# pjmikkol/bwtc

Measured on AMD Instinct MI355X. Metric: MB/s compressed (BWT+encode) on 256 MiB block, higher is better.
Workload: dtype u8/u32/u64 integer

## Files before the change

bwtc_amd/csrc/wavelet_encoder.hip:

```cpp
#include "bwt_engine.hpp"
#include "entropy_host.hpp"
#include "wavelet_host.hpp"
#include "wavelet_pipeline.hpp"
#include <algorithm>
#include <chrono>
#include <future>
#include <cstdio>
#include <cstdlib>
#include <cstring>
#include <map>
#include <memory>
#include <utility>
#include <vector>

namespace bwtc_hip {

static u32 device_model_rejects(const u32* h_tail, u32 n_coded, bool state_ok) {
  u32 r = 0;
  if (h_tail[1]) r |= BWTC_HIP_REJECT_FLAGS;
  if (h_tail[2] != n_coded) r |= BWTC_HIP_REJECT_COUNT;
  if (h_tail[3]) r |= BWTC_HIP_REJECT_SCAN;
  if (!state_ok) r |= BWTC_HIP_REJECT_STATE;
  if (std::getenv("BWTC_HIP_TEST_MODELS_FALLBACK")) r |= BWTC_HIP_REJECT_TEST;
  return r;
// ... 375 lines not shown
    e.prob_free.back()->swap(job.prob);
  }
  *out_bytes = job.record.size();
  const int rc = job.failed ? -2 : job.record.size() <= job.user_cap ? 0 : -1;
  if (e.pipeline) {
    std::shared_ptr<WaveletJob> last(std::move(jobp));
    e.pipeline->dispose(std::move(last));
  }
  return rc;
}

int wavelet_join_begun(BwtEngine& e) {
  if (!e.deferred_queue) return 0;
  for (std::map<u64, std::shared_ptr<DeviceWaveletJob> >::iterator it = e.jobs.begin(); it != e.jobs.end(); ++it) {
    if (it->second->queued) continue;
    const int rc = wavelet_encode_queue(e, it->first, e.wavelet_state, &e.wavelet_state);
    if (rc) return rc;
  }
  return 0;
}

void wavelet_pipeline_release(BwtEngine& e) {
  (void)wavelet_join_begun(e);
  e.half_job.reset();
  e.copy_job.reset();
  for (std::map<u64, std::shared_ptr<DeviceWaveletJob> >::iterator it = e.jobs.begin(); it != e.jobs.end(); ++it)
    if (it->second->queued) HostPipeline::wait(*it->second);
  e.jobs.clear();
  if (e.pipeline && std::getenv("BWTC_HIP_DEBUG") && e.pipeline->clock.blocks)
    std::fprintf(stderr, "wavelet pipeline: %llu blocks; host time in models %.3f s, in range coders %.3f s (summed over threads)\n",
                 (unsigned long long)e.pipeline->clock.blocks.load(), e.pipeline->clock.model_ns.load() * 1e-9,
                 e.pipeline->clock.coder_ns.load() * 1e-9);
  if (e.pipeline && std::getenv("BWTC_HIP_DEBUG") && e.pipeline->clock.scalar_ns.load())
    std::fprintf(stderr, "wavelet pipeline: %.3f s of the range coders' time in the scalar tasks of the longest sections, the rest in the lane engines\n",
                 e.pipeline->clock.scalar_ns.load() * 1e-9);
  delete e.pipeline;
  e.pipeline = nullptr;
  e.codes_pool.clear();
  e.w_pool.clear();
  e.prob_free.clear();
}

}
```

bwtc_amd/csrc/wavelet_pipeline.cpp:

```cpp
#include "wavelet_pipeline.hpp"

#include <algorithm>
#include <cstdio>
#include <cstdlib>
#include <cstring>

namespace bwtc_hip {

namespace {
unsigned envNumber(const char* name, unsigned fallback) {
  const char* v = std::getenv(name);
  return v && std::atoi(v) > 0 ? static_cast<unsigned>(std::atoi(v)) : fallback;
}
uint64_t since(const std::chrono::steady_clock::time_point& t0) {
  return static_cast<uint64_t>(std::chrono::duration_cast<std::chrono::nanoseconds>(std::chrono::steady_clock::now() - t0).count());
}
}

HostPipeline::HostPipeline(unsigned threads, uint64_t huge_group_elements, unsigned depth)
    : groups_(), pool_(threads), huge_(huge_group_elements) {
  const unsigned P = pool_.size();
  const char* force = std::getenv("BWTC_HIP_CODER_LANES");
  const bool lanes = bwtc::wavelet::simdCoderAvailable() && (force ? force[0] == '1' : depth >= kLaneDepth);
  coder_tasks_ = envNumber("BWTC_HIP_CODER_TASKS", 2);
  max_engines_ = std::max(1u, envNumber("BWTC_HIP_MODEL_ENGINES", lanes ? (P * 7 + 15) / 16 : (P + 3) / 4));
  max_coder_engines_ = lanes ? envNumber("BWTC_HIP_CODER_ENGINES", std::max(1u, (P * 6 + 15) / 16)) : 0u;
  long_chain_ = static_cast<uint64_t>(std::getenv("BWTC_HIP_LONG_CHAIN_MI") ? std::atoi(std::getenv("BWTC_HIP_LONG_CHAIN_MI")) : 0) << 20;
  if (std::getenv("BWTC_HIP_LONG_CHAIN_ELEMENTS")) long_chain_ = std::strtoull(std::getenv("BWTC_HIP_LONG_CHAIN_ELEMENTS"), nullptr, 10);
  if (long_chain_ == 0) long_chain_ = ~static_cast<uint64_t>(0);
  max_pair_engines_ = lanes && long_chain_ != ~static_cast<uint64_t>(0) ? envNumber("BWTC_HIP_PAIR_ENGINES", std::max(1u, (P * 3 + 7) / 8)) : 0u;
  const char* fforce = std::getenv("BWTC_HIP_FUSED");
  const bool fused = bwtc::wavelet::simdCoderAvailable() && bwtc::wavelet::simdModelsAvailable() &&
                     (fforce ? fforce[0] == '1' : depth >= kFusedDepth);
  max_fused_engines_ = fused ? envNumber("BWTC_HIP_FUSED_ENGINES", P) : 0u;
  groups_.on_block_modelled = [this](const std::shared_ptr<WaveletJob>& j) { submitSections(j); };
  chains_.on_block_coded = [this](WaveletJob& j) { finish(j); };
  fused_sections_.on_block_coded = [this](WaveletJob& j) { finish(j); };
  long_chains_.on_block_coded = [this](WaveletJob& j) { finish(j); };
  w_chains_.on_block_coded = [this](WaveletJob& j) { finish(j); };
  w_long_chains_.on_block_coded = [this](WaveletJob& j) { finish(j); };
  max_w_engines_ = bwtc::wavelet::simdCoderAvailable() ? envNumber("BWTC_HIP_W_ENGINES", std::max(1u, P / 4)) : 0u;
  if (std::getenv("BWTC_HIP_W_ENGINES") && std::atoi(std::getenv("BWTC_HIP_W_ENGINES")) == 0) max_w_engines_ = 0;
  max_w_pair_engines_ = envNumber("BWTC_HIP_W_PAIR_ENGINES", 0);
  w_lanes_ = envNumber("BWTC_HIP_W_LANES", 16);
  w_long_chain_ = static_cast<uint64_t>(envNumber("BWTC_HIP_W_LONG_MI", 8)) << 20;
  if (std::getenv("BWTC_HIP_LONG_CHAIN_ELEMENTS")) w_long_chain_ = std::strtoull(std::getenv("BWTC_HIP_LONG_CHAIN_ELEMENTS"), nullptr, 10);
}

HostPipeline::~HostPipeline() {}

void HostPipeline::wait(WaveletJob& job) {
  std::unique_lock<std::mutex> g(job.mu);
  job.cv.wait(g, [&] { return job.done; });
}

bool HostPipeline::waitFor(WaveletJob& job, unsigned milliseconds) {
  std::unique_lock<std::mutex> g(job.mu);
  return job.cv.wait_for(g, std::chrono::milliseconds(milliseconds), [&] { return job.done; });
}

void HostPipeline::finishNow(WaveletJob& job) {
  std::vector<uint8_t>& rec = job.record;
  size_t total = rec.size();
  for (size_t s = 0; s < job.outs.size(); ++s) total += job.outs[s].bytes.size();
  rec.reserve(total);
  for (size_t s = 0; s < job.outs.size(); ++s) rec.insert(rec.end(), job.outs[s].bytes.begin(), job.outs[s].bytes.end());
  const uint64_t len = rec.size() - 6;
  for (int i = 0; i < 6; ++i) rec[i] = static_cast<uint8_t>(len >> (8 * (5 - i)));
  if (job.user_out && rec.size() <= job.user_cap) std::memcpy(job.user_out, rec.data(), rec.size());
  job.t_finished = std::chrono::steady_clock::now();
  { std::lock_guard<std::mutex> g(job.mu); job.done = true; job.cv.notify_all(); }
}

void HostPipeline::finish(WaveletJob& job) {
  --clock.unfinished;
  finishNow(job);
  if (job.t_begun.time_since_epoch().count())
    clock.latency_ns += static_cast<uint64_t>(std::chrono::duration_cast<std::chrono::nanoseconds>(job.t_finished - job.t_begun).count());
  ++clock.finished;
// ... 15 lines not shown
  std::vector<std::function<void()> > next;
  const uint64_t longest = std::max<uint64_t>(1, jobp->coder->largestSectionElements());
  const size_t balanced = static_cast<size_t>(std::min<uint64_t>(pool_.size(), jobp->coder->elements() / longest));
  const size_t engines = std::max<size_t>(1, std::min<size_t>(std::max(coder_tasks_, balanced), (jobp->coder->sectionTasks() + 1) / 2));
  for (size_t q = 0; q < engines; ++q) {
    next.push_back([this, jobp] {
      WaveletJob& j = *jobp;
      const auto t0 = std::chrono::steady_clock::now();
      const size_t did = j.coder->codeSectionsPaired(&j.section_cursor, j.prob.data(), &j.outs);
      clock.coder_ns += since(t0);
      bool fin;
      { std::lock_guard<std::mutex> g(j.mu); j.sections_left -= did; fin = did > 0 && j.sections_left == 0; }
      if (fin) finish(j);
    });
  }
  pool_.submit(jobp->rank, next);
}

uint32_t HostPipeline::queue(const std::shared_ptr<WaveletJob>& jobp, uint32_t fsm8_state, char model, const uint32_t* expect_end) {
  WaveletJob& job = *jobp;
  noteBegin();
  if (job.w) {
    job.coder.reset(new bwtc::wavelet::StreamCoder(job.plan, job.coded_pos.data(), job.w_end_state, bwtc::wavelet::StreamCoder::Modelled()));
    freshOutputs(job, job.plan.sections.size());
    job.t_queued = job.t_modelled = std::chrono::steady_clock::now();
    job.models_left = 0;
    job.sections_left = job.coder->sectionTasks();
    ++clock.blocks;
    if (job.sections_left == 0) { finishNow(job); ++clock.finished; return job.w_end_state; }
    ++clock.unfinished;
    if (std::getenv("BWTC_HIP_DEBUG")) {
      std::fprintf(stderr, "w-route: %zu sections, elements (Mi):", job.coder->sectionTasks());
      for (size_t k = 0; k < job.coder->sectionTasks() && k < 12; ++k) std::fprintf(stderr, " %.1f", job.coder->sectionElements(k) / 1048576.0);
      std::fprintf(stderr, " ...; %u lane engines at most, scalar from %.0f Mi\n", max_w_engines_, w_long_chain_ / 1048576.0);
    }
    if (max_w_engines_) {
      const uint64_t cut = std::max<uint64_t>(w_long_chain_, job.coder->largestSectionElements() / 5);
      size_t n_long = 0;
      while (n_long < job.coder->sectionTasks() && job.coder->sectionElements(n_long) >= cut) ++n_long;
      std::vector<std::function<void()> > own;
      if (max_w_pair_engines_ && n_long) {
        if (w_long_chains_.add(jobp, 0, n_long, max_w_pair_engines_))
          pool_.submit(0, [this] { bwtc::wavelet::runCoderLanes(w_long_chains_, 2, &clock.coder_ns); });
      } else
      for (size_t k = 0; k < n_long; ++k) {
        own.push_back([this, jobp, k] {
          WaveletJob& j = *jobp;
          const auto t0 = std::chrono::steady_clock::now();
          j.coder->codeSectionW(k, j.w, &j.outs);
          const uint64_t dt = since(t0);
          clock.coder_ns += dt;
          clock.scalar_ns += dt;
          bool fin;
          { std::lock_guard<std::mutex> g(j.mu); fin = --j.sections_left == 0; }
          if (fin) finish(j);
        });
      }
      if (!own.empty()) pool_.submit(job.rank, own);
      if (w_chains_.add(jobp, n_long, job.coder->sectionTasks(), max_w_engines_))
        pool_.submit(0, [this] { bwtc::wavelet::runCoderLanes(w_chains_, static_cast<int>(w_lanes_), &clock.coder_ns); });
      return job.w_end_state;
    }
    const uint64_t longest = std::max<uint64_t>(1, job.coder->largestSectionElements());
    const size_t balanced = static_cast<size_t>(std::min<uint64_t>(pool_.size(), (job.coder->elements() + longest - 1) / longest));
    const size_t engines = std::max<size_t>(1, std::min<size_t>(std::max<size_t>(2, balanced), job.coder->sectionTasks()));
    std::vector<std::function<void()> > next;
    for (size_t q = 0; q < engines; ++q) {
      next.push_back([this, jobp] {
        WaveletJob& j = *jobp;
        const auto t0 = std::chrono::steady_clock::now();
        const size_t did = j.coder->codeSectionsW(&j.section_cursor, j.w, &j.outs);
        clock.coder_ns += since(t0);
// ... 71 lines not shown
```

bwtc_amd/csrc/wavelet_pipeline.hpp:

```cpp
#pragma once
#include <malloc.h>
#include <atomic>
#include <chrono>
#include <condition_variable>
#include <cstdint>
#include <cstdlib>
#include <deque>
#include <functional>
#include <map>
#include <memory>
#include <mutex>
#include <thread>
#include <vector>

#include <pthread.h>
#include <sched.h>
#include <sys/resource.h>
#include <sys/syscall.h>
#include <unistd.h>

#include "wavelet_host.hpp"

namespace bwtc_hip {

struct StageClock {
  std::atomic<uint64_t> model_ns{0}, coder_ns{0}, blocks{0}, finished{0};
  std::atomic<uint64_t> scalar_ns{0};
  std::atomic<uint64_t> latency_ns{0};
  std::atomic<int> unfinished{0};
};

struct WaveletRoutes {
  std::atomic<uint64_t> trees_device{0}, trees_host{0};
  std::atomic<uint64_t> models_device{0}, models_rejected{0}, lost_turn{0};
// ... 85 lines not shown
  bool next(bwtc::wavelet::ModelGroupDesc* d, int prefer);
  void done(void* cookie);
  bool retire(int prefer) {
    std::lock_guard<std::mutex> g(mu_);
    if (!queue_.empty()) return false;
    --engines_[prefer];
    return true;
  }
  std::function<void(const std::shared_ptr<WaveletJob>&)> on_block_modelled;
 private:
  struct Entry { std::shared_ptr<WaveletJob> job; std::vector<uint32_t> list[2]; size_t at[2]; };
  std::mutex mu_;
  std::deque<Entry> queue_;
  unsigned engines_[3];
};

class BlockChainSource : public bwtc::wavelet::ChainSource {
 public:
  BlockChainSource() : engines_(0) {}
  bool add(const std::shared_ptr<WaveletJob>& job, size_t first, size_t last, unsigned max_engines);
  bool next(bwtc::wavelet::ChainDesc* d);
  void done(void* cookie);
  bool retire() {
    std::lock_guard<std::mutex> g(mu_);
    if (!queue_.empty()) return false;
    --engines_;
    return true;
  }
  std::function<void(WaveletJob&)> on_block_coded;
 private:
  struct Entry { std::shared_ptr<WaveletJob> job; size_t at, end; };
  std::mutex mu_;
  std::deque<Entry> queue_;
  unsigned engines_;
};

class BlockSectionSource : public bwtc::wavelet::SectionSource {
 public:
  BlockSectionSource() : engines_(0) {}
  bool add(const std::shared_ptr<WaveletJob>& job, unsigned max_engines);
  bool next(bwtc::wavelet::FusedSectionDesc* d);
  void done(void* cookie);
  bool retire() {
    std::lock_guard<std::mutex> g(mu_);
    if (!queue_.empty()) return false;
    --engines_;
    return true;
  }
  std::function<void(WaveletJob&)> on_block_coded;
 private:
  struct Entry { std::shared_ptr<WaveletJob> job; size_t at; };
  std::mutex mu_;
  std::deque<Entry> queue_;
  unsigned engines_;
};

struct WaveletJob : std::enable_shared_from_this<WaveletJob> {
  virtual ~WaveletJob() {}
  std::vector<uint8_t> record;
  bwtc::wavelet::StreamPlan plan;
  std::vector<uint32_t> coded_pos;
  const uint8_t* codes = nullptr;
  RawBuffer<uint16_t> prob;
  std::unique_ptr<bwtc::wavelet::StreamCoder> coder;
  std::vector<bwtc::wavelet::SectionOutput> outs;
  std::vector<std::vector<bwtc::wavelet::FusedGroup> > fused_groups;
// ... 68 lines not shown
    const uint64_t now = static_cast<uint64_t>(std::chrono::duration_cast<std::chrono::nanoseconds>(
        std::chrono::steady_clock::now().time_since_epoch()).count());
    const uint64_t last = last_begin_ns_.exchange(now);
    if (last && now > last) {
      const uint64_t d = now - last, old = begin_interval_ns_.load();
      begin_interval_ns_.store(old ? (old * 7 + d) / 8 : d);
    }
  }
  StageClock clock;
  WaveletRoutes* routes = nullptr;
 private:
  std::atomic<uint64_t> last_begin_ns_{0}, begin_interval_ns_{0};
  enum { kSpares = 40 };
  std::atomic<uint32_t> disposed_{0};
  std::mutex spare_mu_;
  std::vector<std::vector<bwtc::wavelet::SectionOutput> > spare_outs_;
  std::vector<std::vector<uint8_t> > spare_records_;
  void freshOutputs(WaveletJob& job, size_t n) {
    if (job.outs.empty()) takeSpareOutputs(&job.outs);
    job.outs.resize(n);
    for (size_t s = 0; s < n; ++s) job.outs[s].bytes.clear();
  }
  void submitSections(const std::shared_ptr<WaveletJob>& job);
  void finish(WaveletJob& job);
  BlockGroupSource groups_;
  BlockChainSource chains_;
  BlockChainSource long_chains_;
  BlockChainSource w_chains_;
  BlockChainSource w_long_chains_;
  unsigned max_w_pair_engines_;
  unsigned w_lanes_;
  unsigned max_w_engines_;
  uint64_t w_long_chain_;
  BlockSectionSource fused_sections_;
  WorkerPool pool_;
  uint64_t huge_;
  unsigned max_engines_;
  unsigned max_coder_engines_;
  unsigned max_pair_engines_;
  uint64_t long_chain_;
  unsigned max_fused_engines_;
  size_t coder_tasks_;
};

inline int BlockGroupSource::add(const std::shared_ptr<WaveletJob>& job, size_t first_group, unsigned max_engines) {
  Entry e;
  e.job = job;
  e.at[0] = e.at[1] = 0;
  for (size_t k = first_group; k < job->coder->modelTasks(); ++k)
    e.list[job->coder->taskIsInteger(k) ? 0 : 1].push_back(static_cast<uint32_t>(k));
  std::lock_guard<std::mutex> g(mu_);
  queue_.push_back(std::move(e));
  if (engines_[1] + engines_[2] >= max_engines) return 0;
  const int prefer = engines_[1] * 2 < engines_[2] || (engines_[2] > 0 && engines_[1] == 0 && max_engines > 1) ? 1 : 2;
  ++engines_[prefer];
  return prefer;
}

inline bool BlockGroupSource::next(bwtc::wavelet::ModelGroupDesc* d, int prefer) {
  std::shared_ptr<WaveletJob> job;
  size_t k = 0;
  {
    std::lock_guard<std::mutex> g(mu_);
    while (!queue_.empty() && queue_.front().at[0] >= queue_.front().list[0].size() &&
           queue_.front().at[1] >= queue_.front().list[1].size())
      queue_.pop_front();
// ... 23 lines not shown
  e.at = first;
  e.end = last;
  std::lock_guard<std::mutex> g(mu_);
  queue_.push_back(std::move(e));
  if (engines_ >= max_engines) return false;
  ++engines_;
  return true;
}

inline bool BlockChainSource::next(bwtc::wavelet::ChainDesc* d) {
  std::shared_ptr<WaveletJob> job;
  size_t k = 0;
  {
    std::lock_guard<std::mutex> g(mu_);
    while (!queue_.empty() && queue_.front().at >= queue_.front().end) queue_.pop_front();
    if (queue_.empty()) return false;
    job = queue_.front().job;
    k = queue_.front().at++;
  }
  if (job->w) job->coder->describeChainW(k, job->w, &job->outs, d);
  else job->coder->describeChain(k, job->prob.data(), &job->outs, d);
  d->cookie = job.get();
  return true;
}

inline void BlockChainSource::done(void* cookie) {
  WaveletJob* job = static_cast<WaveletJob*>(cookie);
  const std::shared_ptr<WaveletJob> keep = job->shared_from_this();
  bool last;
  { std::lock_guard<std::mutex> g(job->mu); last = --job->sections_left == 0; }
  if (last) on_block_coded(*job);
}

inline bool BlockSectionSource::add(const std::shared_ptr<WaveletJob>& job, unsigned max_engines) {
  Entry e;
  e.job = job;
  e.at = 0;
  std::lock_guard<std::mutex> g(mu_);
  queue_.push_back(std::move(e));
  if (engines_ >= max_engines) return false;
  ++engines_;
  return true;
}

inline bool BlockSectionSource::next(bwtc::wavelet::FusedSectionDesc* d) {
  std::shared_ptr<WaveletJob> job;
  size_t k = 0;
  {
    std::lock_guard<std::mutex> g(mu_);
    while (!queue_.empty() && queue_.front().at >= queue_.front().job->coder->sectionTasks()) queue_.pop_front();
    if (queue_.empty()) return false;
    job = queue_.front().job;
    k = queue_.front().at++;
  }
  job->coder->describeSectionFused(k, &job->outs, &job->fused_groups[k], d);
  d->cookie = job.get();
  return true;
}

inline void BlockSectionSource::done(void* cookie) {
  WaveletJob* job = static_cast<WaveletJob*>(cookie);
  const std::shared_ptr<WaveletJob> keep = job->shared_from_this();
  bool last;
  { std::lock_guard<std::mutex> g(job->mu); last = --job->sections_left == 0; }
  if (last) on_block_coded(*job);
}
// ... 10 lines not shown
```

bwtc_amd/csrc/wavelet_rc.cpp:

```cpp
#include "wavelet_rc.hpp"

#include <immintrin.h>

#include <algorithm>
#include <chrono>
#include <cstdlib>
#include <cstring>

namespace bwtc {
namespace wavelet {
namespace {

inline uint32_t codeAt(const uint8_t* codes, uint64_t i) { return (codes[i >> 2] >> ((i & 3) * 2)) & 3u; }

}

void runChain(CoderChain& c, const uint8_t* codes, const uint16_t* prob, uint64_t until) {
  const uint64_t kChunk = 16384;
  uint32_t lo = c.lo, size = c.size;
  uint64_t b = c.i;
  for (; b < until; b += kChunk) {
    const uint64_t ce = std::min(until, b + kChunk);
    uint8_t* o = c.room(kChunk);
#define BWTC_RC_STEP(bit_, p_)                                                                          \
    {                                                                                                    \
      const uint32_t bit = (bit_);                                                                       \
      const uint32_t t = static_cast<uint32_t>((static_cast<uint64_t>(size) * (p_) + 2048u) >> 12);      \
      lo = bit ? lo : lo + t + 1;                                                                        \
      size = bit ? t - 1 : size - t - 1;                                                                 \
      while (((lo ^ (lo + size + 1)) & 0xFF000000u) == 0) { *o++ = static_cast<uint8_t>(lo >> 24); lo <<= 8; size = (size << 8) + 510u; } \
    }
    uint64_t i = b;
    for (; i < ce && (i & 3); ++i) BWTC_RC_STEP(codeAt(codes, i) & 1u, prob[i]);
    for (; i + 4 <= ce; i += 4) {
      const uint32_t four = codes[i >> 2];
      BWTC_RC_STEP(four & 1u, prob[i]);
      BWTC_RC_STEP((four >> 2) & 1u, prob[i + 1]);
      BWTC_RC_STEP((four >> 4) & 1u, prob[i + 2]);
      BWTC_RC_STEP((four >> 6) & 1u, prob[i + 3]);
    }
    for (; i < ce; ++i) BWTC_RC_STEP(codeAt(codes, i) & 1u, prob[i]);
#undef BWTC_RC_STEP
    c.used = static_cast<size_t>(o - c.out->data());
  }
  c.lo = lo; c.size = size; c.i = std::max(c.i, until);
}

void runChainW(CoderChain& c, const uint16_t* w, uint64_t until) {
  const uint64_t kChunk = 16384;
  uint32_t lo = c.lo, size = c.size;
  uint64_t b = c.i;
  for (; b < until; b += kChunk) {
    const uint64_t ce = std::min(until, b + kChunk);
    uint8_t* o = c.room(kChunk);
    for (uint64_t i = b; i < ce; ++i) {
      const uint32_t x = w[i];
      const uint32_t bit = x >> 15, m = x & 0x7FFFu;
      const uint32_t ns = static_cast<uint32_t>((static_cast<int64_t>(static_cast<uint64_t>(size) * m) + (static_cast<int64_t>(bit) - 2049)) >> 12);
      lo += (bit - 1u) & (size - ns);
      size = ns;
      while (((lo ^ (lo + size + 1)) & 0xFF000000u) == 0) { *o++ = static_cast<uint8_t>(lo >> 24); lo <<= 8; size = (size << 8) + 510u; }
    }
    c.used = static_cast<size_t>(o - c.out->data());
  }
  c.lo = lo; c.size = size; c.i = std::max(c.i, until);
}

void runChainPair(CoderChain& a, const uint8_t* codes_a, const uint16_t* prob_a,
                  CoderChain& b, const uint8_t* codes_b, const uint16_t* prob_b, uint64_t limit) {
  const uint64_t kChunk = 8192;
  uint64_t left = std::min(limit, std::min(a.e - a.i, b.e - b.i));
  while (left > 0) {
    const uint64_t n = std::min(left, kChunk);
    uint8_t* oa = a.room(kChunk);
    uint8_t* ob = b.room(kChunk);
    uint32_t loa = a.lo, sa = a.size, lob = b.lo, sb = b.size;
    uint64_t ia = a.i, ib = b.i;
#define BWTC_RC_FREE(lo, size, o, i, codes, prob)                                                         \
    {                                                                                                      \
      const uint32_t bit = codeAt(codes, i) & 1u;                                                          \
      const uint32_t t = static_cast<uint32_t>((static_cast<uint64_t>(size) * prob[i] + 2048u) >> 12);     \
      lo = bit ? lo : lo + t + 1;                                                                          \
      size = bit ? t - 1 : size - t - 1;                                                                   \
      const uint32_t same = ((lo ^ (lo + size + 1)) & 0xFF000000u) == 0;                                   \
      *o = static_cast<uint8_t>(lo >> 24);                                                                 \
      o += same;                                                                                           \
      lo = same ? lo << 8 : lo;                                                                            \
      size = same ? (size << 8) + 510u : size;                                                             \
      while (__builtin_expect(same && ((lo ^ (lo + size + 1)) & 0xFF000000u) == 0, 0)) { *o++ = static_cast<uint8_t>(lo >> 24); lo <<= 8; size = (size << 8) + 510u; } \
      ++i;                                                                                                 \
    }
    for (uint64_t k = 0; k < n; ++k) {
      BWTC_RC_FREE(loa, sa, oa, ia, codes_a, prob_a)
      BWTC_RC_FREE(lob, sb, ob, ib, codes_b, prob_b)
    }
#undef BWTC_RC_FREE
    a.lo = loa; a.size = sa; a.i = ia; a.used = static_cast<size_t>(oa - a.out->data());
    b.lo = lob; b.size = sb; b.i = ib; b.used = static_cast<size_t>(ob - b.out->data());
    left -= n;
  }
}

void runChainPairW(CoderChain& a, const uint16_t* wa, CoderChain& b, const uint16_t* wb, uint64_t limit) {
  const uint64_t kChunk = 8192;
  uint64_t left = std::min(limit, std::min(a.e - a.i, b.e - b.i));
  while (left > 0) {
    const uint64_t n = std::min(left, kChunk);
    uint8_t* oa = a.room(kChunk);
    uint8_t* ob = b.room(kChunk);
    uint32_t loa = a.lo, sa = a.size, lob = b.lo, sb = b.size;
    uint64_t ia = a.i, ib = b.i;
#define BWTC_RC_W(lo, size, o, i, w)                                                                      \
    {                                                                                                      \
      const uint32_t x = w[i];                                                                             \
      const uint32_t bit = x >> 15, m = x & 0x7FFFu;                                                       \
      const uint32_t ns = static_cast<uint32_t>((static_cast<int64_t>(static_cast<uint64_t>(size) * m) + (static_cast<int64_t>(bit) - 2049)) >> 12); \
      lo += (bit - 1u) & (size - ns);                                                                      \
      size = ns;                                                                                           \
      while (((lo ^ (lo + size + 1)) & 0xFF000000u) == 0) { *o++ = static_cast<uint8_t>(lo >> 24); lo <<= 8; size = (size << 8) + 510u; } \
      ++i;                                                                                                 \
    }
    for (uint64_t k = 0; k < n; ++k) {
      BWTC_RC_W(loa, sa, oa, ia, wa)
      BWTC_RC_W(lob, sb, ob, ib, wb)
    }
#undef BWTC_RC_W
    a.lo = loa; a.size = sa; a.i = ia; a.used = static_cast<size_t>(oa - a.out->data());
    b.lo = lob; b.size = sb; b.i = ib; b.used = static_cast<size_t>(ob - b.out->data());
    left -= n;
  }
}

void runChainPair(CoderChain& a, CoderChain& b, const uint8_t* codes, const uint16_t* prob) {
  runChainPair(a, codes, prob, b, codes, prob, ~static_cast<uint64_t>(0));
}

namespace {

const int kLanes = 16;
const uint64_t kScalarOnly = 512;
const int kMinLanes = 4;
const uint64_t kMaxWords = 512;

const int kGroups = 2;
const int kAll = kLanes * kGroups;

struct Lanes {
  alignas(64) uint32_t lo[kAll], size[kAll];
  const uint8_t* codes[kAll];
  const uint16_t* prob[kAll];
  uint64_t i[kAll];
  uint8_t* out[kAll];
  uint32_t advance[kAll];
};

alignas(64) const uint16_t kZeroProb[32] = {0};
alignas(64) const uint8_t kZeroCodes[8] = {0};

#define BWTC_AVX512 __attribute__((target("avx512f,avx512bw,avx512vl,avx512dq")))

BWTC_AVX512 inline void transpose16(__m512i r[16]) {
  __m512i t[16];
  for (int i = 0; i < 16; i += 2) { t[i] = _mm512_unpacklo_epi32(r[i], r[i + 1]); t[i + 1] = _mm512_unpackhi_epi32(r[i], r[i + 1]); }
  for (int i = 0; i < 16; i += 4) {
    r[i] = _mm512_unpacklo_epi64(t[i], t[i + 2]); r[i + 1] = _mm512_unpackhi_epi64(t[i], t[i + 2]);
    r[i + 2] = _mm512_unpacklo_epi64(t[i + 1], t[i + 3]); r[i + 3] = _mm512_unpackhi_epi64(t[i + 1], t[i + 3]);
  }
  for (int i = 0; i < 16; i += 8)
    for (int j = 0; j < 4; ++j) {
      t[i + j] = _mm512_shuffle_i32x4(r[i + j], r[i + j + 4], 0x88);
      t[i + j + 4] = _mm512_shuffle_i32x4(r[i + j], r[i + j + 4], 0xdd);
    }
  for (int j = 0; j < 8; ++j) {
    r[j] = _mm512_shuffle_i32x4(t[j], t[j + 8], 0x88);
    r[j + 8] = _mm512_shuffle_i32x4(t[j], t[j + 8], 0xdd);
  }
}

template <bool WMODE, int G>
BWTC_AVX512 void runWords(Lanes& L, uint64_t words, uint32_t busy_mask) {
  __m512i lo[G], size[G];
  __mmask16 kBusy[G];
  for (int g = 0; g < G; ++g) {
    lo[g] = _mm512_load_si512(L.lo + g * kLanes);
    size[g] = _mm512_load_si512(L.size + g * kLanes);
    kBusy[g] = static_cast<__mmask16>(busy_mask >> (g * kLanes));
  }
  const __m512i one = _mm512_set1_epi32(1), c4095 = _mm512_set1_epi32(4095), c2048 = _mm512_set1_epi32(2048);
  const __m512i top = _mm512_set1_epi32(static_cast<int>(0xFF000000u)), c510 = _mm512_set1_epi32(510);
  const __m512i lane0 = _mm512_slli_epi32(_mm512_setr_epi32(0, 1, 2, 3, 4, 5, 6, 7, 8, 9, 10, 11, 12, 13, 14, 15), 8);
  const __m512i c32768 = _mm512_set1_epi32(32768), c32767 = _mm512_set1_epi32(32767), cm2049 = _mm512_set1_epi32(-2049);
  alignas(64) uint32_t cw[kAll] = {0};
  alignas(64) uint32_t ev[G][16 * kLanes * 4 + 64];
  alignas(64) __m512i P[G][16];
  for (uint64_t w = 0; w < words; ++w) {
    for (int g = 0; g < G; ++g) {
      for (int l = 0; l < kLanes; ++l) {
        const int a = g * kLanes + l;
        P[g][l] = _mm512_cvtepu16_epi32(_mm256_loadu_si256(reinterpret_cast<const __m256i*>(L.prob[a] + L.i[a])));
        if (!WMODE) std::memcpy(&cw[a], L.codes[a] + (L.i[a] >> 2), 4);
        L.i[a] += L.advance[a];
      }
      transpose16(P[g]);
    }
    __m512i W[G];
    uint32_t n[G];
    for (int g = 0; g < G; ++g) { W[g] = _mm512_load_si512(cw + g * kLanes); n[g] = 0; }
    for (int t = 0; t < 16; ++t) {
#pragma GCC unroll 2
      for (int g = 0; g < G; ++g) {
        __m512i p = P[g][t];
        __mmask16 kBit;
        const __m512i hi = _mm512_srli_epi32(size[g], 12), lw = _mm512_and_si512(size[g], c4095);
        if (WMODE) {
          kBit = _mm512_test_epi32_mask(p, c32768);
          const __m512i m = _mm512_and_si512(p, c32767);
          __m512i c = _mm512_add_epi32(_mm512_mullo_epi32(lw, m), cm2049);
          c = _mm512_mask_add_epi32(c, kBit, c, one);
          const __m512i ns = _mm512_add_epi32(_mm512_mullo_epi32(hi, m), _mm512_srai_epi32(c, 12));
          lo[g] = _mm512_mask_add_epi32(lo[g], static_cast<__mmask16>(~kBit), lo[g], _mm512_sub_epi32(size[g], ns));
          size[g] = ns;
        } else {
          kBit = _mm512_test_epi32_mask(W[g], one);
          W[g] = _mm512_srli_epi32(W[g], 2);
          const __m512i tt = _mm512_add_epi32(_mm512_mullo_epi32(hi, p),
                                              _mm512_srli_epi32(_mm512_add_epi32(_mm512_mullo_epi32(lw, p), c2048), 12));
          const __m512i t1 = _mm512_add_epi32(tt, one);
          lo[g] = _mm512_mask_add_epi32(lo[g], static_cast<__mmask16>(~kBit), lo[g], t1);
          size[g] = _mm512_mask_blend_epi32(kBit, _mm512_sub_epi32(size[g], t1), _mm512_sub_epi32(tt, one));
        }
        __m512i hiend = _mm512_add_epi32(_mm512_add_epi32(lo[g], size[g]), one);
        __mmask16 m = _mm512_mask_testn_epi32_mask(kBusy[g], _mm512_xor_si512(lo[g], hiend), top);
        for (;;) {
          _mm512_storeu_si512(ev[g] + n[g], _mm512_maskz_compress_epi32(m, _mm512_or_si512(_mm512_srli_epi32(lo[g], 24), lane0)));
          n[g] += static_cast<uint32_t>(__builtin_popcount(m));
          lo[g] = _mm512_mask_slli_epi32(lo[g], m, lo[g], 8);
          size[g] = _mm512_mask_add_epi32(size[g], m, _mm512_slli_epi32(size[g], 8), c510);
          hiend = _mm512_add_epi32(_mm512_add_epi32(lo[g], size[g]), one);
          m = _mm512_mask_testn_epi32_mask(m, _mm512_xor_si512(lo[g], hiend), top);
          if (__builtin_expect(m == 0, 1)) break;
        }
      }
    }
    for (int g = 0; g < G; ++g)
      for (uint32_t k = 0; k < n[g]; ++k) { const uint32_t e = ev[g][k]; *L.out[g * kLanes + (e >> 8)]++ = static_cast<uint8_t>(e); }
  }
  for (int g = 0; g < G; ++g) {
    _mm512_store_si512(L.lo + g * kLanes, lo[g]);
    _mm512_store_si512(L.size + g * kLanes, size[g]);
  }
}

}

bool simdCoderAvailable() {
  static const bool ok = [] {
    const char* off = std::getenv("BWTC_HIP_SIMD");
    if (off && off[0] == '0') return false;
    off = std::getenv("BWTC_HIP_CODER_LANES");
    if (off && off[0] == '0') return false;
    return __builtin_cpu_supports("avx512f") && __builtin_cpu_supports("avx512bw") &&
           __builtin_cpu_supports("avx512vl") && __builtin_cpu_supports("avx512dq");
  }();
  return ok;
}

void runCoderLanes(ChainSource& src, int max_lanes, std::atomic<uint64_t>* busy_ns) {
  auto tick = std::chrono::steady_clock::now();
  auto account = [&] {
    if (!busy_ns) return;
    const auto now = std::chrono::steady_clock::now();
    *busy_ns += static_cast<uint64_t>(std::chrono::duration_cast<std::chrono::nanoseconds>(now - tick).count());
    tick = now;
  };
  const int lanes = std::max(1, std::min(max_lanes, kAll));
  const bool two = lanes > kLanes;
  Lanes L;
  CoderChain chain[kAll];
  ChainDesc desc[kAll];
  bool busy[kAll];
  for (int l = 0; l < kAll; ++l) busy[l] = false;
  bool sourceDry = false;
  bool wmode = false;
  auto scalar = [&](int l, uint64_t until) {
    if (desc[l].w) runChainW(chain[l], desc[l].w, until); else runChain(chain[l], desc[l].codes, desc[l].prob, until);
  };
  auto finishLane = [&](int l) {
    CoderChain& c = chain[l];
    scalar(l, c.e);
    c.finish();
    src.done(desc[l].cookie);
    busy[l] = false;
  };
  for (;;) {
    int nbusy = 0;
    for (int l = 0; l < lanes; ++l) {
      while (!busy[l] && !sourceDry) {
        if (!src.next(&desc[l])) { sourceDry = true; break; }
        CoderChain& c = chain[l];
        c.start(desc[l].begin, desc[l].end, desc[l].out);
        wmode = desc[l].w != nullptr;
        const uint64_t aligned = (c.i + 15) & ~static_cast<uint64_t>(15);
        busy[l] = true;
        if (c.e - c.i < kScalarOnly || aligned + 16 > c.e) { finishLane(l); continue; }
        scalar(l, aligned);
      }
      nbusy += busy[l];
    }
    account();
    if (nbusy == 0) {
      if (sourceDry && src.retire()) return;
      sourceDry = false;
      continue;
    }
    if (lanes < kMinLanes || (nbusy < kMinLanes && sourceDry)) {
      const uint64_t kSlice = static_cast<uint64_t>(1) << 22;
      int ids[kAll], n = 0;
      for (int l = 0; l < kAll; ++l) if (busy[l]) ids[n++] = l;
      if (n >= 2) {
        const int a = ids[0], b = ids[1];
        if (desc[a].w && desc[b].w) runChainPairW(chain[a], desc[a].w, chain[b], desc[b].w, kSlice);
        else if (desc[a].w || desc[b].w) { scalar(a, std::min(chain[a].e, chain[a].i + kSlice)); scalar(b, std::min(chain[b].e, chain[b].i + kSlice)); }
        else runChainPair(chain[a], desc[a].codes, desc[a].prob, chain[b], desc[b].codes, desc[b].prob, kSlice);
        if (chain[a].i >= chain[a].e) finishLane(a);
        if (chain[b].i >= chain[b].e) finishLane(b);
      } else {
        CoderChain& c = chain[ids[0]];
        scalar(ids[0], std::min(c.e, c.i + kSlice));
        if (c.i >= c.e) finishLane(ids[0]);
      }
      sourceDry = false;
      continue;
    }
    uint64_t words = kMaxWords;
    uint32_t mask = 0;
    for (int l = 0; l < kAll; ++l) if (busy[l]) { words = std::min(words, (chain[l].e - chain[l].i) >> 4); mask |= 1u << l; }
    if (words > 0) {
      for (int l = 0; l < kAll; ++l) {
        if (busy[l]) {
          CoderChain& c = chain[l];
          L.lo[l] = c.lo; L.size[l] = c.size; L.codes[l] = desc[l].codes; L.prob[l] = wmode ? desc[l].w : desc[l].prob; L.i[l] = c.i;
          L.out[l] = c.room(words * 16); L.advance[l] = 16;
        } else {
          L.lo[l] = 0; L.size[l] = 0xFFFFFFFEu; L.codes[l] = kZeroCodes; L.prob[l] = kZeroProb; L.i[l] = 0;
          L.out[l] = nullptr; L.advance[l] = 0;
        }
      }
      if (two && (mask >> kLanes)) { if (wmode) runWords<true, 2>(L, words, mask); else runWords<false, 2>(L, words, mask); }
      else { if (wmode) runWords<true, 1>(L, words, mask); else runWords<false, 1>(L, words, mask); }
      for (int l = 0; l < kAll; ++l) {
        if (!busy[l]) continue;
        CoderChain& c = chain[l];
        c.lo = L.lo[l]; c.size = L.size[l]; c.i = L.i[l];
        c.used = static_cast<size_t>(L.out[l] - c.out->data());
      }
    }
    for (int l = 0; l < kAll; ++l)
      if (busy[l] && chain[l].e - chain[l].i < 16) finishLane(l);
    sourceDry = false;
  }
}

}
}
```

bwtc_amd/csrc/wavelet_rc.hpp:

```cpp
#pragma once
#include <atomic>
#include <cstddef>
#include <cstdint>
#include <vector>

namespace bwtc {
namespace wavelet {

struct CoderChain {
  uint32_t lo, size;
  uint64_t i, e;
  std::vector<uint8_t>* out;
  size_t used;
  void start(uint64_t b, uint64_t end, std::vector<uint8_t>* o) {
    lo = 0; size = 0xFFFFFFFEu; i = b; e = end; out = o; used = o->size();
    if (end - b >= (1u << 16)) o->reserve(used + (end - b) / 7 + 4096);
  }
  uint8_t* room(uint64_t elements) {
    if (out->size() - used < 4 * elements + 8) out->resize(used + 4 * elements + 8 + out->size() / 2);
    return out->data() + used;
  }
  void finish() {
    out->resize(used + 4);
    uint8_t* o = out->data() + used;
    o[0] = static_cast<uint8_t>(lo >> 24); o[1] = 255; o[2] = 255; o[3] = 255;
  }
};

void runChain(CoderChain& c, const uint8_t* codes, const uint16_t* prob, uint64_t until);
void runChainW(CoderChain& c, const uint16_t* w, uint64_t until);
void runChainPairW(CoderChain& a, const uint16_t* wa, CoderChain& b, const uint16_t* wb, uint64_t limit);
void runChainPair(CoderChain& a, CoderChain& b, const uint8_t* codes, const uint16_t* prob);
void runChainPair(CoderChain& a, const uint8_t* codes_a, const uint16_t* prob_a,
                  CoderChain& b, const uint8_t* codes_b, const uint16_t* prob_b, uint64_t limit);

struct ChainDesc {
  const uint8_t* codes;
  const uint16_t* prob;
  uint64_t begin, end;
  std::vector<uint8_t>* out;
  void* cookie;
  const uint16_t* w = nullptr;
};

class ChainSource {
 public:
  virtual ~ChainSource() {}
  virtual bool next(ChainDesc* c) = 0;
  virtual void done(void* cookie) = 0;
  virtual bool retire() { return true; }
};

bool simdCoderAvailable();

void runCoderLanes(ChainSource& src, int max_lanes = 16, std::atomic<uint64_t>* busy_ns = nullptr);

}
}
```

Baseline: 5877.

## Interleave scalar long-chain range coding with AVX-512 lane steps for short sections

```diff
diff --git a/bwtc_amd/csrc/wavelet_encoder.hip b/bwtc_amd/csrc/wavelet_encoder.hip
--- a/bwtc_amd/csrc/wavelet_encoder.hip
+++ b/bwtc_amd/csrc/wavelet_encoder.hip
@@ -431,7 +431,7 @@
                  (unsigned long long)e.pipeline->clock.blocks.load(), e.pipeline->clock.model_ns.load() * 1e-9,
                  e.pipeline->clock.coder_ns.load() * 1e-9);
   if (e.pipeline && std::getenv("BWTC_HIP_DEBUG") && e.pipeline->clock.scalar_ns.load())
-    std::fprintf(stderr, "wavelet pipeline: %.3f s of the range coders' time in the scalar tasks of the longest sections, the rest in the lane engines\n",
+    std::fprintf(stderr, "wavelet pipeline: %.3f s of the range coders' time in the scalar loops of the longest sections (lanes stepped inside them included), the rest in lanes alone\n",
                  e.pipeline->clock.scalar_ns.load() * 1e-9);
   delete e.pipeline;
   e.pipeline = nullptr;
diff --git a/bwtc_amd/csrc/wavelet_pipeline.cpp b/bwtc_amd/csrc/wavelet_pipeline.cpp
--- a/bwtc_amd/csrc/wavelet_pipeline.cpp
+++ b/bwtc_amd/csrc/wavelet_pipeline.cpp
@@ -39,12 +39,17 @@
   long_chains_.on_block_coded = [this](WaveletJob& j) { finish(j); };
   w_chains_.on_block_coded = [this](WaveletJob& j) { finish(j); };
   w_long_chains_.on_block_coded = [this](WaveletJob& j) { finish(j); };
+  w_fused_.on_block_coded = [this](WaveletJob& j) { finish(j); };
   max_w_engines_ = bwtc::wavelet::simdCoderAvailable() ? envNumber("BWTC_HIP_W_ENGINES", std::max(1u, P / 4)) : 0u;
   if (std::getenv("BWTC_HIP_W_ENGINES") && std::atoi(std::getenv("BWTC_HIP_W_ENGINES")) == 0) max_w_engines_ = 0;
   max_w_pair_engines_ = envNumber("BWTC_HIP_W_PAIR_ENGINES", 0);
   w_lanes_ = envNumber("BWTC_HIP_W_LANES", 16);
   w_long_chain_ = static_cast<uint64_t>(envNumber("BWTC_HIP_W_LONG_MI", 8)) << 20;
   if (std::getenv("BWTC_HIP_LONG_CHAIN_ELEMENTS")) w_long_chain_ = std::strtoull(std::getenv("BWTC_HIP_LONG_CHAIN_ELEMENTS"), nullptr, 10);
+  const char* flanes = std::getenv("BWTC_HIP_FUSED_LANES");
+  max_w_fused_engines_ = max_w_engines_ && !(flanes && flanes[0] == '0') && !max_w_pair_engines_
+                             ? envNumber("BWTC_HIP_FUSED_LANES_ENGINES", std::max(1u, P - 1)) : 0u;
+  w_fused_k_ = static_cast<int>(envNumber("BWTC_HIP_FUSED_LANES_K", bwtc::wavelet::kChainLanesK));
 }
 
 HostPipeline::~HostPipeline() {}
@@ -126,12 +131,24 @@
     if (std::getenv("BWTC_HIP_DEBUG")) {
       std::fprintf(stderr, "w-route: %zu sections, elements (Mi):", job.coder->sectionTasks());
       for (size_t k = 0; k < job.coder->sectionTasks() && k < 12; ++k) std::fprintf(stderr, " %.1f", job.coder->sectionElements(k) / 1048576.0);
-      std::fprintf(stderr, " ...; %u lane engines at most, scalar from %.0f Mi\n", max_w_engines_, w_long_chain_ / 1048576.0);
+      if (max_w_fused_engines_)
+        std::fprintf(stderr, " ...; long chains from %.0f Mi with the lanes inside them (a vector step per %d elements), %u engines at most\n",
+                     std::max<uint64_t>(w_long_chain_, job.coder->largestSectionElements() / 5) / 1048576.0, w_fused_k_, max_w_fused_engines_);
+      else
+        std::fprintf(stderr, " ...; %u lane engines at most, scalar from %.0f Mi\n", max_w_engines_, w_long_chain_ / 1048576.0);
     }
     if (max_w_engines_) {
       const uint64_t cut = std::max<uint64_t>(w_long_chain_, job.coder->largestSectionElements() / 5);
       size_t n_long = 0;
       while (n_long < job.coder->sectionTasks() && job.coder->sectionElements(n_long) >= cut) ++n_long;
+      if (max_w_fused_engines_) {
+        const unsigned start = w_fused_.add(jobp, n_long, job.coder->sectionTasks(), max_w_fused_engines_, max_w_engines_);
+        for (unsigned q = 0; q < start; ++q)
+          pool_.submit(0, [this] {
+            bwtc::wavelet::runChainsWithLanes(w_fused_.longs, w_fused_.shorts, w_fused_k_, &clock.coder_ns, &clock.scalar_ns);
+          });
+        return job.w_end_state;
+      }
       std::vector<std::function<void()> > own;
       if (max_w_pair_engines_ && n_long) {
         if (w_long_chains_.add(jobp, 0, n_long, max_w_pair_engines_))
diff --git a/bwtc_amd/csrc/wavelet_pipeline.hpp b/bwtc_amd/csrc/wavelet_pipeline.hpp
--- a/bwtc_amd/csrc/wavelet_pipeline.hpp
+++ b/bwtc_amd/csrc/wavelet_pipeline.hpp
@@ -1,5 +1,6 @@
 #pragma once
 #include <malloc.h>
+#include <algorithm>
 #include <atomic>
 #include <chrono>
 #include <condition_variable>
@@ -151,6 +152,35 @@
   struct Entry { std::shared_ptr<WaveletJob> job; size_t at, end; };
   std::mutex mu_;
   std::deque<Entry> queue_;
+  unsigned engines_;
+};
+
+class BlockLongShortSource {
+ public:
+  BlockLongShortSource() : longs(this, 0), shorts(this, 1), engines_(0) {}
+  unsigned add(const std::shared_ptr<WaveletJob>& job, size_t n_long, size_t n, unsigned max_engines, unsigned max_lane_engines);
+  struct Side : bwtc::wavelet::ChainSource {
+    Side(BlockLongShortSource* s, int k) : src(s), kind(k) {}
+    bool next(bwtc::wavelet::ChainDesc* d) { return src->next(kind, d); }
+    void done(void* cookie) { src->done(cookie); }
+    bool retire() { return src->retire(); }
+    BlockLongShortSource* src;
+    int kind;
+  };
+  Side longs, shorts;
+  std::function<void(WaveletJob&)> on_block_coded;
+ private:
+  struct Entry { std::shared_ptr<WaveletJob> job; size_t at, end; };
+  bool next(int kind, bwtc::wavelet::ChainDesc* d);
+  void done(void* cookie);
+  bool retire() {
+    std::lock_guard<std::mutex> g(mu_);
+    if (!queue_[0].empty() || !queue_[1].empty()) return false;
+    --engines_;
+    return true;
+  }
+  std::mutex mu_;
+  std::deque<Entry> queue_[2];
   unsigned engines_;
 };
 
@@ -285,6 +315,9 @@
   unsigned w_lanes_;
   unsigned max_w_engines_;
   uint64_t w_long_chain_;
+  BlockLongShortSource w_fused_;
+  unsigned max_w_fused_engines_;
+  int w_fused_k_;
   BlockSectionSource fused_sections_;
   WorkerPool pool_;
   uint64_t huge_;
@@ -374,6 +407,42 @@
   if (last) on_block_coded(*job);
 }
 
+inline unsigned BlockLongShortSource::add(const std::shared_ptr<WaveletJob>& job, size_t n_long, size_t n, unsigned max_engines,
+                                          unsigned max_lane_engines) {
+  std::lock_guard<std::mutex> g(mu_);
+  if (n_long > 0) { Entry e; e.job = job; e.at = 0; e.end = n_long; queue_[0].push_back(std::move(e)); }
+  if (n > n_long) { Entry e; e.job = job; e.at = n_long; e.end = n; queue_[1].push_back(std::move(e)); }
+  const unsigned limit = std::max(1u, n_long > 0 ? max_engines : std::min(max_engines, max_lane_engines));
+  const unsigned want = static_cast<unsigned>(std::max<size_t>(1, n_long));
+  const unsigned start = engines_ >= limit ? 0u : std::min(want, limit - engines_);
+  engines_ += start;
+  return start;
+}
+
+inline bool BlockLongShortSource::next(int kind, bwtc::wavelet::ChainDesc* d) {
+  std::shared_ptr<WaveletJob> job;
+  size_t k = 0;
+  {
+    std::lock_guard<std::mutex> g(mu_);
+    std::deque<Entry>& q = queue_[kind];
+    while (!q.empty() && q.front().at >= q.front().end) q.pop_front();
+    if (q.empty()) return false;
+    job = q.front().job;
+    k = q.front().at++;
+  }
+  job->coder->describeChainW(k, job->w, &job->outs, d);
+  d->cookie = job.get();
+  return true;
+}
+
+inline void BlockLongShortSource::done(void* cookie) {
+  WaveletJob* job = static_cast<WaveletJob*>(cookie);
+  const std::shared_ptr<WaveletJob> keep = job->shared_from_this();
+  bool last;
+  { std::lock_guard<std::mutex> g(job->mu); last = --job->sections_left == 0; }
+  if (last) on_block_coded(*job);
+}
+
 inline bool BlockSectionSource::add(const std::shared_ptr<WaveletJob>& job, unsigned max_engines) {
   Entry e;
   e.job = job;
diff --git a/bwtc_amd/csrc/wavelet_rc.cpp b/bwtc_amd/csrc/wavelet_rc.cpp
--- a/bwtc_amd/csrc/wavelet_rc.cpp
+++ b/bwtc_amd/csrc/wavelet_rc.cpp
@@ -12,6 +12,14 @@
 namespace {
 
 inline uint32_t codeAt(const uint8_t* codes, uint64_t i) { return (codes[i >> 2] >> ((i & 3) * 2)) & 3u; }
+
+__attribute__((always_inline)) inline void stepW(uint32_t& lo, uint32_t& size, uint8_t*& o, uint32_t x) {
+  const uint32_t bit = x >> 15, m = x & 0x7FFFu;
+  const uint32_t ns = static_cast<uint32_t>((static_cast<int64_t>(static_cast<uint64_t>(size) * m) + (static_cast<int64_t>(bit) - 2049)) >> 12);
+  lo += (bit - 1u) & (size - ns);
+  size = ns;
+  while (((lo ^ (lo + size + 1)) & 0xFF000000u) == 0) { *o++ = static_cast<uint8_t>(lo >> 24); lo <<= 8; size = (size << 8) + 510u; }
+}
 
 }
 
@@ -53,14 +61,7 @@
   for (; b < until; b += kChunk) {
     const uint64_t ce = std::min(until, b + kChunk);
     uint8_t* o = c.room(kChunk);
-    for (uint64_t i = b; i < ce; ++i) {
-      const uint32_t x = w[i];
-      const uint32_t bit = x >> 15, m = x & 0x7FFFu;
-      const uint32_t ns = static_cast<uint32_t>((static_cast<int64_t>(static_cast<uint64_t>(size) * m) + (static_cast<int64_t>(bit) - 2049)) >> 12);
-      lo += (bit - 1u) & (size - ns);
-      size = ns;
-      while (((lo ^ (lo + size + 1)) & 0xFF000000u) == 0) { *o++ = static_cast<uint8_t>(lo >> 24); lo <<= 8; size = (size << 8) + 510u; }
-    }
+    for (uint64_t i = b; i < ce; ++i) stepW(lo, size, o, w[i]);
     c.used = static_cast<size_t>(o - c.out->data());
   }
   c.lo = lo; c.size = size; c.i = std::max(c.i, until);
@@ -110,21 +111,10 @@
     uint8_t* ob = b.room(kChunk);
     uint32_t loa = a.lo, sa = a.size, lob = b.lo, sb = b.size;
     uint64_t ia = a.i, ib = b.i;
-#define BWTC_RC_W(lo, size, o, i, w)                                                                      \
-    {                                                                                                      \
-      const uint32_t x = w[i];                                                                             \
-      const uint32_t bit = x >> 15, m = x & 0x7FFFu;                                                       \
-      const uint32_t ns = static_cast<uint32_t>((static_cast<int64_t>(static_cast<uint64_t>(size) * m) + (static_cast<int64_t>(bit) - 2049)) >> 12); \
-      lo += (bit - 1u) & (size - ns);                                                                      \
-      size = ns;                                                                                           \
-      while (((lo ^ (lo + size + 1)) & 0xFF000000u) == 0) { *o++ = static_cast<uint8_t>(lo >> 24); lo <<= 8; size = (size << 8) + 510u; } \
-      ++i;                                                                                                 \
-    }
     for (uint64_t k = 0; k < n; ++k) {
-      BWTC_RC_W(loa, sa, oa, ia, wa)
-      BWTC_RC_W(lob, sb, ob, ib, wb)
-    }
-#undef BWTC_RC_W
+      stepW(loa, sa, oa, wa[ia++]);
+      stepW(lob, sb, ob, wb[ib++]);
+    }
     a.lo = loa; a.size = sa; a.i = ia; a.used = static_cast<size_t>(oa - a.out->data());
     b.lo = lob; b.size = sb; b.i = ib; b.used = static_cast<size_t>(ob - b.out->data());
     left -= n;
@@ -177,8 +167,14 @@
   }
 }
 
-template <bool WMODE, int G>
-BWTC_AVX512 void runWords(Lanes& L, uint64_t words, uint32_t busy_mask) {
+struct Rider {
+  uint32_t lo, size;
+  const uint16_t* x;
+  uint8_t* o;
+};
+
+template <bool WMODE, int G, int K = 0>
+BWTC_AVX512 void runWords(Lanes& L, uint64_t words, uint32_t busy_mask, Rider* rider = nullptr) {
   __m512i lo[G], size[G];
   __mmask16 kBusy[G];
   for (int g = 0; g < G; ++g) {
@@ -193,6 +189,10 @@
   alignas(64) uint32_t cw[kAll] = {0};
   alignas(64) uint32_t ev[G][16 * kLanes * 4 + 64];
   alignas(64) __m512i P[G][16];
+  uint32_t rlo = 0, rsize = 0;
+  const uint16_t* rx = nullptr;
+  uint8_t* ro = nullptr;
+  if (K > 0) { rlo = rider->lo; rsize = rider->size; rx = rider->x; ro = rider->o; }
   for (uint64_t w = 0; w < words; ++w) {
     for (int g = 0; g < G; ++g) {
       for (int l = 0; l < kLanes; ++l) {
@@ -241,6 +241,10 @@
           if (__builtin_expect(m == 0, 1)) break;
         }
       }
+      if (K > 0) {
+        for (int k = 0; k < K; ++k) stepW(rlo, rsize, ro, rx[k]);
+        rx += K;
+      }
     }
     for (int g = 0; g < G; ++g)
       for (uint32_t k = 0; k < n[g]; ++k) { const uint32_t e = ev[g][k]; *L.out[g * kLanes + (e >> 8)]++ = static_cast<uint8_t>(e); }
@@ -249,7 +253,90 @@
     _mm512_store_si512(L.lo + g * kLanes, lo[g]);
     _mm512_store_si512(L.size + g * kLanes, size[g]);
   }
-}
+  if (K > 0) { rider->lo = rlo; rider->size = rsize; rider->x = rx; rider->o = ro; }
+}
+
+struct LaneSet {
+  CoderChain chain[kAll];
+  ChainDesc desc[kAll];
+  bool busy[kAll];
+  bool wmode = false;
+  ChainSource& src;
+  explicit LaneSet(ChainSource& s) : src(s) { for (int l = 0; l < kAll; ++l) busy[l] = false; }
+
+  void scalar(int l, uint64_t until) {
+    if (desc[l].w) runChainW(chain[l], desc[l].w, until); else runChain(chain[l], desc[l].codes, desc[l].prob, until);
+  }
+  void finishLane(int l) {
+    CoderChain& c = chain[l];
+    scalar(l, c.e);
+    c.finish();
+    src.done(desc[l].cookie);
+    busy[l] = false;
+  }
+  int refill(int lanes, bool* dry, uint32_t* mask) {
+    int nbusy = 0;
+    *mask = 0;
+    for (int l = 0; l < lanes; ++l) {
+      while (!busy[l] && !*dry) {
+        if (!src.next(&desc[l])) { *dry = true; break; }
+        CoderChain& c = chain[l];
+        c.start(desc[l].begin, desc[l].end, desc[l].out);
+        wmode = desc[l].w != nullptr;
+        const uint64_t aligned = (c.i + 15) & ~static_cast<uint64_t>(15);
+        busy[l] = true;
+        if (c.e - c.i < kScalarOnly || aligned + 16 > c.e) { finishLane(l); continue; }
+        scalar(l, aligned);
+      }
+      if (busy[l]) { ++nbusy; *mask |= 1u << l; }
+    }
+    return nbusy;
+  }
+  uint64_t words(uint64_t limit) const {
+    for (int l = 0; l < kAll; ++l) if (busy[l]) limit = std::min(limit, (chain[l].e - chain[l].i) >> 4);
+    return limit;
+  }
+  void toVectors(Lanes& L, uint64_t words) {
+    for (int l = 0; l < kAll; ++l) {
+      if (busy[l]) {
+        CoderChain& c = chain[l];
+        L.lo[l] = c.lo; L.size[l] = c.size; L.codes[l] = desc[l].codes; L.prob[l] = wmode ? desc[l].w : desc[l].prob; L.i[l] = c.i;
+        L.out[l] = c.room(words * 16); L.advance[l] = 16;
+      } else {
+        L.lo[l] = 0; L.size[l] = 0xFFFFFFFEu; L.codes[l] = kZeroCodes; L.prob[l] = kZeroProb; L.i[l] = 0;
+        L.out[l] = nullptr; L.advance[l] = 0;
+      }
+    }
+  }
+  void fromVectors(const Lanes& L) {
+    for (int l = 0; l < kAll; ++l) {
+      if (!busy[l]) continue;
+      CoderChain& c = chain[l];
+      c.lo = L.lo[l]; c.size = L.size[l]; c.i = L.i[l];
+      c.used = static_cast<size_t>(L.out[l] - c.out->data());
+    }
+  }
+  void finishTails() {
+    for (int l = 0; l < kAll; ++l)
+      if (busy[l] && chain[l].e - chain[l].i < 16) finishLane(l);
+  }
+  void scalarSlice(uint64_t slice) {
+    int ids[kAll], n = 0;
+    for (int l = 0; l < kAll; ++l) if (busy[l]) ids[n++] = l;
+    if (n >= 2) {
+      const int a = ids[0], b = ids[1];
+      if (desc[a].w && desc[b].w) runChainPairW(chain[a], desc[a].w, chain[b], desc[b].w, slice);
+      else if (desc[a].w || desc[b].w) { scalar(a, std::min(chain[a].e, chain[a].i + slice)); scalar(b, std::min(chain[b].e, chain[b].i + slice)); }
+      else runChainPair(chain[a], desc[a].codes, desc[a].prob, chain[b], desc[b].codes, desc[b].prob, slice);
+      if (chain[a].i >= chain[a].e) finishLane(a);
+      if (chain[b].i >= chain[b].e) finishLane(b);
+    } else {
+      CoderChain& c = chain[ids[0]];
+      scalar(ids[0], std::min(c.e, c.i + slice));
+      if (c.i >= c.e) finishLane(ids[0]);
+    }
+  }
+};
 
 }
 
@@ -276,37 +363,11 @@
   const int lanes = std::max(1, std::min(max_lanes, kAll));
   const bool two = lanes > kLanes;
   Lanes L;
-  CoderChain chain[kAll];
-  ChainDesc desc[kAll];
-  bool busy[kAll];
-  for (int l = 0; l < kAll; ++l) busy[l] = false;
+  LaneSet S(src);
   bool sourceDry = false;
-  bool wmode = false;
-  auto scalar = [&](int l, uint64_t until) {
-    if (desc[l].w) runChainW(chain[l], desc[l].w, until); else runChain(chain[l], desc[l].codes, desc[l].prob, until);
-  };
-  auto finishLane = [&](int l) {
-    CoderChain& c = chain[l];
-    scalar(l, c.e);
-    c.finish();
-    src.done(desc[l].cookie);
-    busy[l] = false;
-  };
   for (;;) {
-    int nbusy = 0;
-    for (int l = 0; l < lanes; ++l) {
-      while (!busy[l] && !sourceDry) {
-        if (!src.next(&desc[l])) { sourceDry = true; break; }
-        CoderChain& c = chain[l];
-        c.start(desc[l].begin, desc[l].end, desc[l].out);
-        wmode = desc[l].w != nullptr;
-        const uint64_t aligned = (c.i + 15) & ~static_cast<uint64_t>(15);
-        busy[l] = true;
-        if (c.e - c.i < kScalarOnly || aligned + 16 > c.e) { finishLane(l); continue; }
-        scalar(l, aligned);
-      }
-      nbusy += busy[l];
-    }
+    uint32_t mask = 0;
+    const int nbusy = S.refill(lanes, &sourceDry, &mask);
     account();
     if (nbusy == 0) {
       if (sourceDry && src.retire()) return;
@@ -314,49 +375,88 @@
       continue;
     }
     if (lanes < kMinLanes || (nbusy < kMinLanes && sourceDry)) {
-      const uint64_t kSlice = static_cast<uint64_t>(1) << 22;
-      int ids[kAll], n = 0;
-      for (int l = 0; l < kAll; ++l) if (busy[l]) ids[n++] = l;
-      if (n >= 2) {
-        const int a = ids[0], b = ids[1];
-        if (desc[a].w && desc[b].w) runChainPairW(chain[a], desc[a].w, chain[b], desc[b].w, kSlice);
-        else if (desc[a].w || desc[b].w) { scalar(a, std::min(chain[a].e, chain[a].i + kSlice)); scalar(b, std::min(chain[b].e, chain[b].i + kSlice)); }
-        else runChainPair(chain[a], desc[a].codes, desc[a].prob, chain[b], desc[b].codes, desc[b].prob, kSlice);
-        if (chain[a].i >= chain[a].e) finishLane(a);
-        if (chain[b].i >= chain[b].e) finishLane(b);
-      } else {
-        CoderChain& c = chain[ids[0]];
-        scalar(ids[0], std::min(c.e, c.i + kSlice));
-        if (c.i >= c.e) finishLane(ids[0]);
-      }
+      S.scalarSlice(static_cast<uint64_t>(1) << 22);
       sourceDry = false;
       continue;
     }
-    uint64_t words = kMaxWords;
+    const uint64_t words = S.words(kMaxWords);
+    if (words > 0) {
+      S.toVectors(L, words);
+      if (two && (mask >> kLanes)) { if (S.wmode) runWords<true, 2>(L, words, mask); else runWords<false, 2>(L, words, mask); }
+      else { if (S.wmode) runWords<true, 1>(L, words, mask); else runWords<false, 1>(L, words, mask); }
+      S.fromVectors(L);
+    }
+    S.finishTails();
+    sourceDry = false;
+  }
+}
+
+void runChainsWithLanes(ChainSource& longs, ChainSource& lanes, int k, std::atomic<uint64_t>* busy_ns, std::atomic<uint64_t>* long_ns) {
+  auto tick = std::chrono::steady_clock::now();
+  auto account = [&](bool holding) {
+    if (!busy_ns && !long_ns) return;
+    const auto now = std::chrono::steady_clock::now();
+    const uint64_t dt = static_cast<uint64_t>(std::chrono::duration_cast<std::chrono::nanoseconds>(now - tick).count());
+    if (busy_ns) *busy_ns += dt;
+    if (holding && long_ns) *long_ns += dt;
+    tick = now;
+  };
+  const int K = k <= 4 ? 4 : k == 5 ? 5 : k <= 6 ? 6 : 8;
+  const uint64_t perWord = 16u * static_cast<uint64_t>(K);
+  const uint64_t kSlice = static_cast<uint64_t>(1) << 20;
+  Lanes L;
+  LaneSet S(lanes);
+  CoderChain lc;
+  ChainDesc ld;
+  bool holding = false, sourceDry = false;
+  for (;;) {
+    if (!holding && longs.next(&ld)) {
+      account(false);
+      lc.start(ld.begin, ld.end, ld.out);
+      holding = true;
+    }
     uint32_t mask = 0;
-    for (int l = 0; l < kAll; ++l) if (busy[l]) { words = std::min(words, (chain[l].e - chain[l].i) >> 4); mask |= 1u << l; }
-    if (words > 0) {
-      for (int l = 0; l < kAll; ++l) {
-        if (busy[l]) {
-          CoderChain& c = chain[l];
-          L.lo[l] = c.lo; L.size[l] = c.size; L.codes[l] = desc[l].codes; L.prob[l] = wmode ? desc[l].w : desc[l].prob; L.i[l] = c.i;
-          L.out[l] = c.room(words * 16); L.advance[l] = 16;
-        } else {
-          L.lo[l] = 0; L.size[l] = 0xFFFFFFFEu; L.codes[l] = kZeroCodes; L.prob[l] = kZeroProb; L.i[l] = 0;
-          L.out[l] = nullptr; L.advance[l] = 0;
+    const int nbusy = S.refill(kLanes, &sourceDry, &mask);
+    if (holding) {
+      const uint64_t left = lc.e - lc.i;
+      if (nbusy == 0 || left < perWord) {
+        runChainW(lc, ld.w, nbusy ? lc.e : std::min(lc.e, lc.i + kSlice));
+      } else {
+        const uint64_t words = S.words(std::min(kMaxWords, left / perWord));
+        S.toVectors(L, words);
+        Rider r;
+        r.lo = lc.lo; r.size = lc.size; r.x = ld.w + lc.i; r.o = lc.room(words * perWord);
+        switch (K) {
+          case 4: runWords<true, 1, 4>(L, words, mask, &r); break;
+          case 5: runWords<true, 1, 5>(L, words, mask, &r); break;
+          case 6: runWords<true, 1, 6>(L, words, mask, &r); break;
+          default: runWords<true, 1, 8>(L, words, mask, &r); break;
         }
-      }
-      if (two && (mask >> kLanes)) { if (wmode) runWords<true, 2>(L, words, mask); else runWords<false, 2>(L, words, mask); }
-      else { if (wmode) runWords<true, 1>(L, words, mask); else runWords<false, 1>(L, words, mask); }
-      for (int l = 0; l < kAll; ++l) {
-        if (!busy[l]) continue;
-        CoderChain& c = chain[l];
-        c.lo = L.lo[l]; c.size = L.size[l]; c.i = L.i[l];
-        c.used = static_cast<size_t>(L.out[l] - c.out->data());
-      }
-    }
-    for (int l = 0; l < kAll; ++l)
-      if (busy[l] && chain[l].e - chain[l].i < 16) finishLane(l);
+        lc.lo = r.lo; lc.size = r.size; lc.i += words * perWord;
+        lc.used = static_cast<size_t>(r.o - lc.out->data());
+        S.fromVectors(L);
+      }
+      if (lc.i >= lc.e) {
+        lc.finish();
+        account(true);
+        holding = false;
+        longs.done(ld.cookie);
+      }
+    } else if (nbusy == 0) {
+      account(false);
+      if (sourceDry && longs.retire()) return;
+      sourceDry = false;
+      continue;
+    } else if (nbusy < kMinLanes && sourceDry) {
+      S.scalarSlice(kSlice);
+    } else {
+      const uint64_t words = S.words(kMaxWords);
+      S.toVectors(L, words);
+      runWords<true, 1>(L, words, mask);
+      S.fromVectors(L);
+    }
+    S.finishTails();
+    account(holding);
     sourceDry = false;
   }
 }
diff --git a/bwtc_amd/csrc/wavelet_rc.hpp b/bwtc_amd/csrc/wavelet_rc.hpp
--- a/bwtc_amd/csrc/wavelet_rc.hpp
+++ b/bwtc_amd/csrc/wavelet_rc.hpp
@@ -55,5 +55,9 @@
 
 void runCoderLanes(ChainSource& src, int max_lanes = 16, std::atomic<uint64_t>* busy_ns = nullptr);
 
+const int kChainLanesK = 6;
+void runChainsWithLanes(ChainSource& longs, ChainSource& lanes, int k = kChainLanesK,
+                        std::atomic<uint64_t>* busy_ns = nullptr, std::atomic<uint64_t>* long_ns = nullptr);
+
 }
 }
```

New measurement: 6948, median of 6. 1.18x the previous value.
